# KrishTanna28/Real-Time-Video-Deepfake-Detection

Hardware: AMD Instinct MI355X
Metric: face-crops/sec (224x224 crops through EfficientNet-B0 classify) (higher is better)
Workload: dtype f32; 1 GPU; configs[1]: batch=256 random 224x224 crops, EfficientNet-B0 fp32 inference; batch_per_gpu=256, parallelism=frame-shard x1, no data-path collective, forwards_in_flight=2

## Files before the change

### real-time-video-deepfake-detection_amd/csrc/b0_kernels.h

```cpp
#pragma once
#include <hip/hip_runtime.h>

#include <string>

namespace dfd {

typedef __bf16 bf16_t;

enum Act { ACT_NONE = 0, ACT_SWISH = 1, ACT_RELU = 2, ACT_PRELU = 3 };

template <typename XT>
void launch_stem(const float* x_nchw, const float* w , const float* b,
                 XT* y, int n, hipStream_t s);

template <typename XT>
void launch_stem_dw(const float* x_nchw, const unsigned short* ws3, int plane, int Kp, const float* bs, const float* Wd,
                    const float* bd, XT* Y, float* P, XT* stem_out, int n, int* tiles, hipStream_t s);

void launch_pointwise(const float* X, const float* W, const float* bias, const float* gate,
                      const float* R, float* Y, int M, int K, int N, int HW, int act,
                      hipStream_t s);

struct ConvGeom {
    int H = 0, W = 0, Ho = 0, Wo = 0, Cin = 0, ksize = 1, stride = 1, pad = 0, dil = 1;
// ... 2 lines not shown
bool launch_conv_gemm(const float* X, const float* W, const float* bias, const float* R, float* Y,
                      int n_img, const ConvGeom& g, int Cout, int act, bool res_first, hipStream_t s);

size_t split_weights_count(int N, int K);
void launch_split_weights(const float* W, unsigned short* out, int N, int K, hipStream_t s, bool transposed = false);
bool split_gemm_supports(int K, int N);
bool split_gemm_thin_supports(int K, int N, int HW);
struct S6Table;
S6Table* s6_table_create();
void s6_table_destroy(S6Table* t);
void s6_table_set_force(S6Table* t, int idx);
void s6_table_set_tuning(S6Table* t, bool on);
int s6_table_measured(const S6Table* t);
int s6_max_candidates();
long long s6_chunk_rows(long long M, long long row_bytes, long long HW);
std::string s6_table_export(const S6Table* t);
int s6_table_import(S6Table* t, const char* text, size_t len);
template <typename XT>
bool launch_pointwise_split(S6Table* tab, const XT* X, const unsigned short* W3, const float* bias, const float* gate,
                            const XT* R, XT* Y, int M, int K, int N, int HW, int act, int planes, hipStream_t s);
template <typename XT>
bool launch_conv_gemm_split(S6Table* tab, const XT* X, const unsigned short* W3, const float* bias, const XT* R,
                            XT* Y, int n_img, const ConvGeom& g, int Cout, int act, bool res_first, int planes, hipStream_t s);

template <typename XT>
bool launch_depthwise(const XT* X, const float* W , const float* bias, XT* Y,
                      float* P, int n, int H, int C, int k, int stride, int pad_lo,
                      int* tiles, hipStream_t s);
int depthwise_tiles(int H, int C, int k, int stride);
template <typename XT>
bool launch_mbconv_front(const XT* Xin, int Cin, const unsigned short* We3, int plane, int Kp, const float* Wef, const float* be,
                         const float* Wd, const float* bd, XT* Y, float* P, int n, int H, int C, int k, int stride,
                         int pad_lo, int* tiles, hipStream_t s, bool late = false);
int mbconv_tiles(int H, int C, int k, int stride, int Cin, bool late = false);

void launch_se(const float* P, int tiles, float inv_hw, const float* w1, const float* b1,
               const float* w2t, const float* b2, float* gate, int n, int C, int c_se,
               hipStream_t s);

template <typename XT>
void launch_avgpool(const XT* X, float* Y, int n, int hw, int C, hipStream_t s);
void launch_bf16_to_f32(const bf16_t* x, float* y, size_t n, hipStream_t s);

}
```

### real-time-video-deepfake-detection_amd/csrc/b0_kernels.hip

```cpp
#include "b0_kernels.h"
#include "kernel_util.h"

#include <cstdlib>

namespace dfd {

#ifdef MB_TRACE
__device__ long long g_mb_trace[256];
#define MB_TP(id)                                                                                             \
    do {                                                                                                      \
        if (H == MB_TRACE_H && S == MB_TRACE_S && bid.x == 5 && bid.n == 3 && threadIdx.x == 0 && mtp < 250) { \
            g_mb_trace[mtp++] = (long long)(id);                                                              \
            g_mb_trace[mtp++] = (long long)__builtin_amdgcn_s_memtime();                                      \
        }                                                                                                     \
    } while (0)
#ifndef MB_TRACE_H
#define MB_TRACE_H 56
#endif
#ifndef MB_TRACE_S
#define MB_TRACE_S 1
#endif
extern "C" int dfd_debug_mb_trace(long long* out, int n) {
    return (int)hipMemcpyFromSymbol(out, HIP_SYMBOL(g_mb_trace), (size_t)n * sizeof(long long), 0, hipMemcpyDeviceToHost);
}
// ... 399 lines not shown
    __shared__ v4f wl[K * K * CG];
    __shared__ v4f red[4 * CG];
    const int tid = threadIdx.x;
    const BlkId bid = blk_image_major(tiles_sp * (C / CB));
    const int n = bid.n;
    const int t = bid.x % tiles_sp, chunk = bid.x / tiles_sp;
    const int ty0 = (t / tiles_x) * TH, tx0 = (t % tiles_x) * TW, c0 = chunk * CB;
    const v4f bv = ldg4(bias + c0 + 4 * (tid % CG));
    for (int i = tid; i < K * K * CG; i += 256)
        wl[i] = ldg4(Wt + (size_t)(i / CG) * C + c0 + 4 * (i % CG));
    const int iy0 = ty0 * S - pad_lo, ix0 = tx0 * S - pad_lo;
    const XT* xb = X + (size_t)n * H * H * C + c0;
    constexpr int NEL = IH * IW * CG, NLD = (NEL + 255) / 256;
    v4f stg[NLD];
    bool stg_ok[NLD];
#pragma unroll
    for (int k = 0; k < NLD; ++k) {
        const int i = tid + k * 256 < NEL ? tid + k * 256 : NEL - 1;
        const int cg = i % CG, pix = i / CG;
        const int iy = iy0 + pix / IW, ix = ix0 + pix % IW;
        const bool inside = (unsigned)iy < (unsigned)H && (unsigned)ix < (unsigned)H;
        stg[k] = ld4(xb + ((size_t)(inside ? iy : 0) * H + (inside ? ix : 0)) * C + 4 * cg);
        stg_ok[k] = inside;
    }
#pragma unroll
    for (int k = 0; k < NLD; ++k) {
        const int i = tid + k * 256 < NEL ? tid + k * 256 : NEL - 1;
        tile[i] = stg_ok[k] ? stg[k] : (v4f){0.f, 0.f, 0.f, 0.f};
    }
    __syncthreads();
    dw_compute<K, S, CB, TH, TW, RP, false, XT>(tile, wl, red, bv, Y, P, n, Ho, C, c0, ty0, tx0, t, tiles_sp);
}

template <int K, int S, int CB, int TH, int TW, int RP, int KC, int NSUB, typename XT, int CI>
__global__ __launch_bounds__(256, ((S == 1 && (((TH - 1) * S + K) * ((TW - 1) * S + K) + 63) / 64 * KC > 12) ? 2 : 3)) void mbconv_kernel(const XT* __restrict__ X,
                                                     const float* __restrict__ We,
                                                     const float* __restrict__ be,
                                                     const float* __restrict__ Wt,
                                                     const float* __restrict__ bias,
                                                     XT* __restrict__ Y, float* __restrict__ P,
                                                     int H, int Ho, int C, int Cin, int pad_lo,
                                                     int tiles_x, int tiles_sp) {
    using Sh = DwShape<K, S, CB, TH, TW>;
    constexpr int CG = Sh::CG, IH = Sh::IH, IW = Sh::IW;
    constexpr int NTB = CB / 16;
    constexpr int NP = IH * IW, NMT = (NP + 15) / 16, NIT = (NMT + 3) / 4;
    constexpr int NM = CI / 4;
    static_assert(sizeof(XT) == 4 && CI % 8 == 0 && KC == (NM + 3) / 4, "fp32 activations, compile-time Cin");
    __shared__ v4f tile[IH * IW * CG];
    __shared__ v4f wl[K * K * CG];
    __shared__ v4f red[4 * CG];
    const int tid = threadIdx.x, lane = tid & 63, wave = tid >> 6, j = lane & 15, q = lane >> 4;
    const BlkId bid = blk_image_major(tiles_sp * (C / (CB * NSUB)));
    const int n = bid.n;
    const int t = bid.x % tiles_sp, group = bid.x / tiles_sp;
    const int ty0 = (t / tiles_x) * TH, tx0 = (t % tiles_x) * TW;
    const int iy0 = ty0 * S - pad_lo, ix0 = tx0 * S - pad_lo;
#ifdef MB_TRACE
    int mtp = 0;
#endif
    MB_TP(0);

    const XT* xb = X + (size_t)n * H * H * Cin;
    v4f xf[NIT][KC];
#pragma unroll
    for (int it = 0; it < NIT; ++it) {
        const int p = (wave + 4 * it) * 16 + j;
        const int iy = iy0 + p / IW, ix = ix0 + p % IW;
        const bool inside = p < NP && (unsigned)iy < (unsigned)H && (unsigned)ix < (unsigned)H;
        const float* px = reinterpret_cast<const float*>(xb) + ((size_t)(inside ? iy : 0) * H + (inside ? ix : 0)) * CI + q * NM;
#pragma unroll
        for (int kk = 0; kk < KC; ++kk) {
            v4f v;
            if (NM % 4 == 0 || kk < KC - 1) v = ldg4u(px + 4 * kk);
            else { const v2f t2 = ldg2(px + 4 * kk); v = (v4f){t2.x, t2.y, 0.f, 0.f}; }
            xf[it][kk] = inside ? v : (v4f){0.f, 0.f, 0.f, 0.f};
        }
    }

    static_assert(K * K * CG <= 256, "one depthwise weight vector per thread");
    struct ChunkW { v4f wl, bv, wf[NTB][KC], bex[NTB]; };
    auto load_chunk = [&](int sub, ChunkW& w) {
        const int c0 = (group * NSUB + sub) * CB;
        const int i = tid < K * K * CG ? tid : 0;
        w.wl = ldg4(Wt + (size_t)(i / CG) * C + c0 + 4 * (i % CG));
        w.bv = ldg4(bias + c0 + 4 * (tid % CG));
#pragma unroll
        for (int nt = 0; nt < NTB; ++nt) {
            w.bex[nt] = ldg4(be + c0 + nt * 16 + 4 * q);
#pragma unroll
            for (int kk = 0; kk < KC; ++kk) {
                const float* pw = We + (size_t)(c0 + nt * 16 + j) * CI + q * NM + 4 * kk;
                if (NM % 4 == 0 || kk < KC - 1) w.wf[nt][kk] = ldg4u(pw);
                else { const v2f t2 = ldg2(pw); w.wf[nt][kk] = (v4f){t2.x, t2.y, 0.f, 0.f}; }
            }
        }
    };
    ChunkW cw[2];
    load_chunk(0, cw[0]);
#pragma unroll
    for (int sub = 0; sub < NSUB; ++sub) {
        const int c0 = (group * NSUB + sub) * CB;
        ChunkW& cur = cw[sub & 1];
        MB_TP(1);
        if (sub > 0) __syncthreads();
        MB_TP(2);
        if (tid < K * K * CG) wl[tid] = cur.wl;
        load_chunk(sub + 1 < NSUB ? sub + 1 : NSUB - 1, cw[(sub + 1) & 1]);
        const v4f bv = cur.bv;
        v4f (&wf)[NTB][KC] = cur.wf;
        v4f (&bex)[NTB] = cur.bex;
        MB_TP(3);
#pragma unroll
        for (int it = 0; it < NIT; ++it) {
            const int mt = wave + 4 * it;
            if (mt < NMT) {
                v4f acc[NTB];
#pragma unroll
                for (int nt = 0; nt < NTB; ++nt) acc[nt] = bex[nt];
                if constexpr (NTB == 1) {
                    v4f acc1 = (v4f){0.f, 0.f, 0.f, 0.f};
#pragma unroll
                    for (int i = 0; i < NM; ++i) {
                        if (i & 1) acc1 = __builtin_amdgcn_mfma_f32_16x16x4f32(wf[0][i / 4][i % 4], xf[it][i / 4][i % 4], acc1, 0, 0, 0);
                        else acc[0] = __builtin_amdgcn_mfma_f32_16x16x4f32(wf[0][i / 4][i % 4], xf[it][i / 4][i % 4], acc[0], 0, 0, 0);
                    }
                    acc[0] += acc1;
                } else {
#pragma unroll
                    for (int i = 0; i < NM; ++i)
#pragma unroll
                        for (int nt = 0; nt < NTB; ++nt)
// ... 326 lines not shown
    }
    MB_TP(4);
    __syncthreads();
    MB_TP(5);
    dw_compute<K, S, CB, TH, TW, RP, false, XT>(tile, wl, red, bv, Y, P, n, 112, 32, 0, ty0, tx0, t, tiles_sp);
    MB_TP(6);
#ifdef MB_TRACE
    if (bid.x == 5 && bid.n == 3 && threadIdx.x == 0) g_mb_trace[255] = mtp;
#endif
}

template <typename XT>
void launch_stem_dw(const float* x, const unsigned short* ws3, int plane, int Kp, const float* bs, const float* Wd,
                    const float* bd, XT* Y, float* P, XT* stem_out, int n, int* tiles, hipStream_t s) {
    const int tx = 112 / 16, ty = 112 / 8;
    *tiles = tx * ty;
    hipLaunchKernelGGL(stem_dw_kernel<XT>, dim3(tx * ty * n), dim3(256), 0, s, x, ws3, plane, Kp, bs, Wd, bd, Y, P, stem_out, tx,
                       tx * ty);
}
template void launch_stem_dw<float>(const float*, const unsigned short*, int, int, const float*, const float*, const float*, float*, float*, float*, int, int*, hipStream_t);
template void launch_stem_dw<bf16_t>(const float*, const unsigned short*, int, int, const float*, const float*, const float*, bf16_t*, float*, bf16_t*, int, int*, hipStream_t);

template <int K, int S, int CB, int TH, int TW, int RP, typename XT>
static void dw_launch(const XT* X, const float* W, const float* b, XT* Y, float* P, int n,
                      int H, int C, int pad_lo, int* tiles, hipStream_t s) {
    const int Ho = (H + S - 1) / S;
    const int tx = (Ho + TW - 1) / TW, ty = (Ho + TH - 1) / TH;
    const int tiles_sp = tx * ty;
    *tiles = tiles_sp;
    hipLaunchKernelGGL((dw_kernel<K, S, CB, TH, TW, RP, XT>), dim3(tiles_sp * (C / CB) * n), dim3(256), 0,
                       s, X, W, b, Y, P, H, Ho, C, pad_lo, tx, tiles_sp);
}

template <int K, int S, int CB, int TH, int TW, int RP, int KC, int NSUB, typename XT, int CI>
static void mb_launch(const XT* X, int Cin, const float* We, const float* be, const float* W, const float* b,
                      XT* Y, float* P, int n, int H, int C, int pad_lo, int* tiles, hipStream_t s) {
    const int Ho = (H + S - 1) / S;
    const int tx = (Ho + TW - 1) / TW, ty = (Ho + TH - 1) / TH;
    const int tiles_sp = tx * ty;
    *tiles = tiles_sp;
    hipLaunchKernelGGL((mbconv_kernel<K, S, CB, TH, TW, RP, KC, NSUB, XT, CI>), dim3(tiles_sp * (C / (CB * NSUB)) * n),
                       dim3(256), 0, s, X, We, be, W, b, Y, P, H, Ho, C, Cin, pad_lo, tx, tiles_sp);
}


template <int K, int CPT, typename XT>
__global__ __launch_bounds__(256) void dw_rows7_kernel(const XT* __restrict__ X, const float* __restrict__ Wt,
                                                       const float* __restrict__ bias, XT* __restrict__ Y,
                                                       float* __restrict__ P, int C, int groups) {
    constexpr int H = 7, PAD = (K - 1) / 2, NV = CPT / 4;
    __shared__ v4f red[8 * 32 * NV];
    const BlkId bid = blk_image_major(groups);
    const int tid = threadIdx.x, row = tid >> 5, cl = tid & 31;
    const int c = (bid.x * 32 + cl) * CPT;
    const bool live = row < H && c < C;
    const int cc = c < C ? c : 0, r = row < H ? row : 0;
    const XT* xb = X + (size_t)bid.n * H * H * C + cc;
    v4f acc[H][NV];
#pragma unroll
    for (int v = 0; v < NV; ++v) {
        const v4f bv = ldg4(bias + cc + 4 * v);
#pragma unroll
        for (int ox = 0; ox < H; ++ox) acc[ox][v] = bv;
    }
    constexpr int KY_UNROLL = K == 3 && CPT == 4 ? 3 : (CPT == 4 ? 2 : 1);
#pragma unroll KY_UNROLL
    for (int ky = 0; ky < K; ++ky) {
        const int iy = r + ky - PAD;
        const bool ok = (unsigned)iy < (unsigned)H;
        const XT* xr = xb + (size_t)(ok ? iy : 0) * H * C;
        v4f in[H][NV], w[K][NV];
#pragma unroll
        for (int ix = 0; ix < H; ++ix)
#pragma unroll
            for (int v = 0; v < NV; ++v) in[ix][v] = ld4(xr + (size_t)ix * C + 4 * v);
// ... 447 lines not shown
    }
    if (var == 17 && k == 5 && stride == 1 && H == 28 && C == 240 && Cin == 40) {
        mb2_launch<5, 1, 16, 14, 28, 4, 2, XT, 256, false, 40, 4>(Xin, Cin, We3, plane, Kp, Wef, be, Wd, bd, Y, P, n, H, C, pad_lo, tiles, s);
        return true;
    }
    if (var == 14 && k == 5 && stride == 1 && H == 28 && C == 240 && Cin == 40) {
        mb2_launch<5, 1, 16, 7, 28, 7, 2, XT, 256, false, 40, 4>(Xin, Cin, We3, plane, Kp, Wef, be, Wd, bd, Y, P, n, H, C, pad_lo, tiles, s);
        return true;
    }
    if (var == 13 && k == 3 && stride == 1 && H == 56 && C == 144 && Cin == 24) {
        mb2_launch<3, 1, 16, 14, 28, 7, 1, XT, 256, true, 24, 4>(Xin, Cin, We3, plane, Kp, Wef, be, Wd, bd, Y, P, n, H, C, pad_lo, tiles, s);
        return true;
    }
#ifdef DFD_MB_ABLATION
#define DFD_ABL_CASE(A)                                                                                              \
    if (var == 20 + A && H == 56 && stride == 1) {                                                                  \
        const int tx = 2, ty = 4;                                                                                   \
        *tiles = tx * ty;                                                                                           \
        hipLaunchKernelGGL((mbconv2_kernel<3, 1, 16, 14, 28, 7, 1, XT, A, 256, false, 24>), dim3(tx * ty * (C / 16) * n), dim3(256), 0, s, Xin, \
                           We3, plane, Kp, Wef, be, Wd, bd, Y, P, H, 56, C, Cin, pad_lo, tx, tx * ty);              \
        return true;                                                                                                \
    }                                                                                                               \
    if (var == 20 + A && H == 28 && stride == 1) {                                                                  \
        *tiles = 1;                                                                                                 \
        hipLaunchKernelGGL((mbconv2_kernel<5, 1, 16, 28, 28, 7, 2, XT, A, 256, false, 40>), dim3((C / 16) * n), dim3(256), 0, s, Xin,   \
                           We3, plane, Kp, Wef, be, Wd, bd, Y, P, H, 28, C, Cin, pad_lo, 1, 1);                     \
        return true;                                                                                                \
    }
    DFD_MB2_ABL(DFD_ABL_CASE)
#undef DFD_ABL_CASE
#endif
    return false;
}
template bool launch_mbconv_front<float>(const float*, int, const unsigned short*, int, int, const float*, const float*, const float*, const float*, float*, float*, int, int, int, int, int, int, int*, hipStream_t, bool);
template bool launch_mbconv_front<bf16_t>(const bf16_t*, int, const unsigned short*, int, int, const float*, const float*, const float*, const float*, bf16_t*, float*, int, int, int, int, int, int, int*, hipStream_t, bool);

int mbconv_tiles(int H, int C, int k, int stride, int Cin, bool late) {
    const int Ho = (H + stride - 1) / stride;
    int best = -1;
#define DFD_MB2_TILES(VV, KK, SS, HH, CC, CI, CB, TH, TW, RP, NK)                    \
    if (k == KK && stride == SS && H == HH && C == CC && Cin == CI) {                \
        const int tl = ((Ho + TW - 1) / TW) * ((Ho + TH - 1) / TH);                  \
        if (tl > best) best = tl;                                                    \
    }
    DFD_MB2_TABLE(DFD_MB2_TILES)
#define DFD_MB3_TILES(VV, KK, SS, HH, CC, CI, CB, TH, TW, RP, NK, NT, INS) DFD_MB2_TILES(VV, KK, SS, HH, CC, CI, CB, TH, TW, RP, NK)
    DFD_MB3_TABLE(DFD_MB3_TILES)
#undef DFD_MB3_TILES
#undef DFD_MB2_TILES
#define DFD_MB1_TILES(VV, KK, SS, HH, CC, CI, CB, TH, TW, RP, KC, NSUB)              \
    if (k == KK && stride == SS && H == HH && C == CC && Cin == CI) {                \
        const int tl = ((Ho + TW - 1) / TW) * ((Ho + TH - 1) / TH);                  \
        if (tl > best) best = tl;                                                    \
    }
    DFD_MB1_TABLE(DFD_MB1_TILES)
#undef DFD_MB1_TILES
    if (k == 5 && stride == 1 && H == 28 && C == 240 && Cin == 40 && best < 4) best = 4;
#define DFD_MB_LATE_TILES(KK, SS, HH, CC, CI) \
    if (late && k == KK && stride == SS && H == HH && C == CC && Cin == CI && best < 1) best = 1;
    DFD_MB_LATE_TABLE(DFD_MB_LATE_TILES)
#undef DFD_MB_LATE_TILES
    return best;
}

int depthwise_tiles(int H, int C, int k, int stride) {
    const int Ho = (H + stride - 1) / stride;
// ... 129 lines not shown
```

### real-time-video-deepfake-detection_amd/csrc/b0_plan.hip

```cpp
#include <algorithm>

#include "b0_kernels.h"
#include "dfd_common.h"

namespace dfd {

thread_local std::string g_create_error;

int fail(dfd_handle* h, int code, const char* fmt, ...) {
    char buf[512];
    va_list ap;
    va_start(ap, fmt);
    vsnprintf(buf, sizeof buf, fmt, ap);
    va_end(ap);
    if (h) h->err = buf;
    else g_create_error = buf;
    return code;
}

namespace {

struct Stage { int rep, k, s, e, ci, co; };
const Stage kStages[] = {{1, 3, 1, 1, 32, 16}, {2, 3, 2, 6, 16, 24}, {2, 5, 2, 6, 24, 40},
                         {3, 3, 2, 6, 40, 80}, {3, 5, 1, 6, 80, 112}, {4, 5, 2, 6, 112, 192},
// ... 156 lines not shown
    return pool.emplace(key, key).first->second.c_str();
}

}

template <typename XT>
static int b0_forward_t(dfd_handle* h, const float* x, int n, float* logits_dev, B0Tap* tap, B0Prof* prof) {
    if (n <= 0) return fail(h, DFD_ERR_ARG, "batch must be positive");
    if (n > h->max_batch) return fail(h, DFD_ERR_CAPACITY, "batch %d exceeds handle capacity %d", n, h->max_batch);
    const B0Plan& P = h->b0;
    hipStream_t s = h->stream;
    Marks mk{prof, s};
    int rc;
    XT* const io0 = reinterpret_cast<XT*>(h->io0);
    XT* const io1 = reinterpret_cast<XT*>(h->io1);
    XT* const expbuf = reinterpret_cast<XT*>(h->expbuf);
    XT* const dwbuf = reinterpret_cast<XT*>(h->dwbuf);
    XT* const headbuf = reinterpret_cast<XT*>(h->headbuf);
    mk.mark("start");
    const bool stem_fused = h->fuse_stem && P.blocks[0].expand == 1;
    int stem_tiles = 0;
    if (stem_fused) {
        const bool want_stem = tap && tap->name && std::string(tap->name) == "stem";
        const unsigned short* ws3 = split_weights(h, P.stem_w, 32, 27, true);
        if (!ws3) return DFD_ERR_HIP;
        launch_stem_dw<XT>(x, ws3, (int)split_weights_count(32, 27), 64, P.stem_b, P.blocks[0].dw_w, P.blocks[0].dw_b, dwbuf,
                           h->pool, want_stem ? io0 : (XT*)nullptr, n, &stem_tiles, s);
        mk.mark("b0.dw");
    } else {
        launch_stem<XT>(x, P.stem_w, P.stem_b, io0, n, s);
        mk.mark("stem");
    }
    if ((rc = tap_out(h, tap, "stem", io0, (size_t)n * 112 * 112 * 32))) return rc;
    XT* cur = io0;
    XT* nxt = io1;
    int bi = 0;
    for (const B0Block& b : P.blocks) {
        const int m_in = n * b.h_in * b.h_in, m_out = n * b.h_out * b.h_out;
        const std::string q = "b" + std::to_string(bi);
        const XT* dw_in = cur;
        int tiles = 0;
        bool fused = false;
        const unsigned short* we3 = nullptr;
        const bool late_here = h->fuse_late && !((h->fuse_late_skip >> bi) & 1u);
        if (b.expand != 1 && h->fuse_expand && mbconv_tiles(b.h_in, b.c_exp, b.kernel, b.stride, b.c_in, late_here) > 0 &&
            !(we3 = split_weights(h, b.exp_w, b.c_exp, b.c_in))) return DFD_ERR_HIP;
        if (we3 && launch_mbconv_front<XT>(cur, b.c_in, we3, (int)split_weights_count(b.c_exp, b.c_in), (b.c_in + 63) / 64 * 64,
                                           b.exp_w, b.exp_b, b.dw_w, b.dw_b, dwbuf, h->pool, n, b.h_in, b.c_exp,
                                           b.kernel, b.stride, b.pad_lo, &tiles, s, late_here)) {
            fused = true;
            mk.mark(layer_name(bi, "dw"));
            if (tap && tap->name && q + ".exp" == tap->name)
                return fail(h, DFD_ERR_STATE, "tap '%s': the expanded tensor is not materialised when expand is fused "
                                              "(dfd_set_option(h, \"fuse_expand\", 0))", tap->name);
        }
        if (!fused && b.expand != 1) {
            if ((rc = pointwise_t<XT>(h, cur, b.exp_w, b.exp_b, nullptr, nullptr, expbuf, m_in, b.c_in, b.c_exp,
                                      b.h_in * b.h_in, ACT_SWISH))) return rc;
            mk.mark(layer_name(bi, "exp"));
            if ((rc = tap_out(h, tap, q + ".exp", expbuf, (size_t)m_in * b.c_exp))) return rc;
            dw_in = expbuf;
        }
        if (bi == 0 && stem_fused) {
            tiles = stem_tiles;
        } else if (!fused) {
            if (!launch_depthwise<XT>(dw_in, b.dw_w, b.dw_b, dwbuf, h->pool, n, b.h_in, b.c_exp, b.kernel,
                                      b.stride, b.pad_lo, &tiles, s))
                return fail(h, DFD_ERR_STATE, "no depthwise kernel for block %d", bi);
            mk.mark(layer_name(bi, "dw"));
        }
        if ((rc = tap_out(h, tap, q + ".dw", dwbuf, (size_t)m_out * b.c_exp))) return rc;
        launch_se(h->pool, tiles, 1.0f / (float)(b.h_out * b.h_out), b.se_w1, b.se_b1, b.se_w2, b.se_b2,
                  h->gate, n, b.c_exp, b.c_se, s);
        mk.mark(layer_name(bi, "se"));
        if ((rc = tap_out(h, tap, q + ".gate", h->gate, (size_t)n * b.c_exp))) return rc;
        if ((rc = pointwise_t<XT>(h, dwbuf, b.proj_w, b.proj_b, h->gate, b.skip ? cur : (const XT*)nullptr, nxt, m_out,
                                  b.c_exp, b.c_out, b.h_out * b.h_out, ACT_NONE))) return rc;
        mk.mark(layer_name(bi, "proj"));
        if ((rc = tap_out(h, tap, q + ".out", nxt, (size_t)m_out * b.c_out))) return rc;
        XT* t = cur; cur = nxt; nxt = t;
        ++bi;
    }
    const B0Block& last = P.blocks.back();
    const int hw = last.h_out * last.h_out;
    if ((rc = pointwise_t<XT>(h, cur, P.head_w, P.head_b, nullptr, nullptr, headbuf, n * hw, last.c_out, 1280, hw,
                              ACT_SWISH))) return rc;
    mk.mark("head");
    if ((rc = tap_out(h, tap, "head", headbuf, (size_t)n * hw * 1280))) return rc;
    launch_avgpool<XT>(headbuf, h->feat, n, hw, 1280, s);
    mk.mark("avgpool");
    if ((rc = tap_out(h, tap, "feat", h->feat, (size_t)n * 1280))) return rc;
    if (!logits_dev) return DFD_OK;
    if ((rc = pointwise(h, h->feat, P.fc1_w, P.fc1_b, nullptr, nullptr, h->fc1, n, 1280, 512, 1, ACT_RELU))) return rc;
    if ((rc = pointwise(h, h->fc1, P.fc2_w, P.fc2_b, nullptr, nullptr, h->fc2, n, 512, 256, 1, ACT_RELU))) return rc;
    launch_pointwise(h->fc2, P.fc3_w, P.fc3_b, nullptr, nullptr, logits_dev, n, 256, 1, 1, ACT_NONE, s);
    mk.mark("mlp");
    if ((rc = tap_out(h, tap, "logit", logits_dev, (size_t)n))) return rc;
    DFD_HIP_TRY(h, hipGetLastError());
    return DFD_OK;
}

float* b0_last_block_out(const dfd_handle* h) { return h->b0.blocks.size() % 2 == 0 ? h->io0 : h->io1; }

int b0_head_preact(dfd_handle* h, int n, void* z_out) {
    const B0Plan& P = h->b0;
    const B0Block& last = P.blocks.back();
    const int hw = last.h_out * last.h_out;
    if (h->act_bf16)
        return pointwise_t<bf16_t>(h, reinterpret_cast<const bf16_t*>(b0_last_block_out(h)), P.head_w, P.head_b, nullptr, nullptr,
                                   static_cast<bf16_t*>(z_out), n * hw, last.c_out, 1280, hw, ACT_NONE);
    return pointwise_t<float>(h, b0_last_block_out(h), P.head_w, P.head_b, nullptr, nullptr, static_cast<float*>(z_out),
                              n * hw, last.c_out, 1280, hw, ACT_NONE);
// ... 10 lines not shown
```

### real-time-video-deepfake-detection_amd/csrc/dfd_api.hip

```cpp
#include "b0_kernels.h"
#include "dfd_common.h"

using namespace dfd;

namespace {

int dev_alloc(dfd_handle* h, size_t bytes, float** out) {
    void* p = nullptr;
    DFD_HIP_TRY(h, hipMalloc(&p, bytes ? bytes : 4));
    h->owned.push_back(p);
    *out = static_cast<float*>(p);
    return DFD_OK;
}

__global__ __launch_bounds__(256) void fill_pattern_kernel(float* __restrict__ x, size_t n) {
    const size_t i = (size_t)blockIdx.x * 256 + threadIdx.x;
    if (i >= n) return;
    uint32_t v = (uint32_t)i * 2654435761u;
    v ^= v >> 15; v *= 2246822519u; v ^= v >> 13;
    x[i] = ((float)(v >> 8) * (1.0f / 16777216.0f) - 0.5f) * 4.0f;
}

int create_impl(dfd_handle* h, int device, const void* blob, size_t blob_len, int max_batch) {
    int ndev = 0;
    if (hipGetDeviceCount(&ndev) != hipSuccess || ndev <= 0)
        return fail(h, DFD_ERR_NO_DEVICE, "no HIP device visible (this library has no CPU path)");
    if (device < 0 || device >= ndev) return fail(h, DFD_ERR_ARG, "device %d out of range (0..%d)", device, ndev - 1);
    DFD_HIP_TRY(h, hipSetDevice(device));
    hipDeviceProp_t prop;
    DFD_HIP_TRY(h, hipGetDeviceProperties(&prop, device));
    if (strncmp(prop.gcnArchName, "gfx950", 6) != 0)
        return fail(h, DFD_ERR_NO_DEVICE, "device %d is %s; this library is built for gfx950 only", device, prop.gcnArchName);
    h->device = device;
    h->max_batch = max_batch;
    if (const char* e = getenv("DFD_FUSE_EXPAND")) h->fuse_expand = atoi(e) != 0;
    if (const char* e = getenv("DFD_FUSE_STEM")) h->fuse_stem = atoi(e) != 0;
    if (const char* e = getenv("DFD_FUSE_LATE")) h->fuse_late = atoi(e) != 0;
    if (const char* e = getenv("DFD_FUSE_LATE_SKIP")) h->fuse_late_skip = (unsigned)atoi(e);
    if (const char* e = getenv("DFD_SPLIT_GEMM")) h->split_gemm = atoi(e) != 0;
    if (const char* e = getenv("DFD_BF16_ACTIVATIONS")) h->act_bf16 = atoi(e) != 0;
    if (const char* e = getenv("DFD_JPEG_DEVICE_RESTART")) h->jpeg_device_restart = atoi(e) != 0;
    h->gemm = s6_table_create();
    if (!h->gemm) return fail(h, DFD_ERR_ARG, "out of host memory");
    DFD_HIP_TRY(h, hipStreamCreateWithFlags(&h->stream, hipStreamNonBlocking));
    DFD_HIP_TRY(h, hipEventCreate(&h->ev0));
    DFD_HIP_TRY(h, hipEventCreate(&h->ev1));

    std::string perr;
    if (!parse_blob(blob, blob_len, &h->tensors, &perr)) return fail(h, DFD_ERR_BLOB, "%s", perr.c_str());
    size_t total = 0;
    for (auto& kv : h->tensors) total += (kv.second.count * 4 + 255) / 256 * 256;
    float* wbase = nullptr;
    int rc = dev_alloc(h, total, &wbase);
    if (rc) return rc;
    size_t off = 0;
    for (auto& kv : h->tensors) {
        Tensor& t = kv.second;
        t.dev = reinterpret_cast<float*>(reinterpret_cast<char*>(wbase) + off);
        DFD_HIP_TRY(h, hipMemcpy(t.dev, t.host, t.count * 4, hipMemcpyHostToDevice));
        t.host = nullptr;
        off += (t.count * 4 + 255) / 256 * 256;
    }
    if ((rc = b0_build_plan(h))) return rc;
    if ((rc = color_tables_init(h))) return rc;
    if ((rc = ssd_init(h))) return rc;
    if ((rc = mtcnn_init(h))) return rc;
    if ((rc = haar_init(h))) return rc;

    const B0Plan& P = h->b0;
// ... 60 lines not shown
extern "C" {

int dfd_abi_version(void) { return DFD_ABI_VERSION; }

int dfd_create(int device, const void* blob, size_t blob_len, int max_batch, dfd_handle** out) {
    if (!out) return fail(nullptr, DFD_ERR_ARG, "dfd_create: out is null");
    *out = nullptr;
    if (!blob || max_batch <= 0 || max_batch > 4096)
        return fail(nullptr, DFD_ERR_ARG, "dfd_create: blob is null or max_batch outside 1..4096");
    dfd_handle* h = new (std::nothrow) dfd_handle();
    if (!h) return fail(nullptr, DFD_ERR_ARG, "dfd_create: out of host memory");
    const int rc = create_impl(h, device, blob, blob_len, max_batch);
    if (rc != DFD_OK) {
        g_create_error = h->err;
        destroy_impl(h);
        return rc;
    }
    *out = h;
    return DFD_OK;
}

void dfd_destroy(dfd_handle* h) { destroy_impl(h); }

const char* dfd_last_error(const dfd_handle* h) { return h ? h->err.c_str() : g_create_error.c_str(); }

int dfd_max_batch(const dfd_handle* h) { return h ? h->max_batch : DFD_ERR_ARG; }

int dfd_set_option(dfd_handle* h, const char* name, int value) {
    if (!h || !name) return DFD_ERR_ARG;
    if (strcmp(name, "fuse_expand") == 0) { h->fuse_expand = value != 0; return DFD_OK; }
    if (strcmp(name, "fuse_late") == 0) { h->fuse_late = value != 0; return DFD_OK; }
    if (strcmp(name, "fuse_late_skip") == 0) { h->fuse_late_skip = (unsigned)value; return DFD_OK; }
    if (strcmp(name, "fuse_stem") == 0) { h->fuse_stem = value != 0; return DFD_OK; }
    if (strcmp(name, "split_gemm") == 0) { h->split_gemm = value != 0; return DFD_OK; }
    if (strcmp(name, "mtcnn") == 0) { h->use_mtcnn = value != 0; return DFD_OK; }
    if (strcmp(name, "overlap_forensics") == 0) { h->overlap_forensics = value != 0; return DFD_OK; }
    if (strcmp(name, "bf16_activations") == 0) { h->act_bf16 = value != 0; return DFD_OK; }
    if (strcmp(name, "bf16_weight_planes") == 0) {
        if (value != 1 && value != 3) return fail(h, DFD_ERR_ARG, "bf16_weight_planes must be 1 or 3");
        h->bf16_planes = value;
        return DFD_OK;
    }
    if (strcmp(name, "gemm_tile") == 0) { s6_table_set_force(h->gemm, value); return DFD_OK; }
    if (strcmp(name, "jpeg_device_entropy") == 0) { h->jpeg_device_entropy = value < 0 ? 0 : value; return DFD_OK; }
    if (strcmp(name, "jpeg_device_restart") == 0) { h->jpeg_device_restart = value != 0; return DFD_OK; }
    if (strcmp(name, "jpeg_rounds") == 0) { h->jpeg_rounds = value; return DFD_OK; }
    if (strcmp(name, "jpeg_chunk_bytes") == 0) {
        if (value < 256 || value > (1 << 20) || (value & (value - 1))) return fail(h, DFD_ERR_ARG, "jpeg_chunk_bytes: a power of two in 256 .. 2^20");
        h->jpeg_chunk_bytes = value;
        return DFD_OK;
    }
    if (strcmp(name, "stream_priority") == 0) {
        if (value < -1 || value > 1) return fail(h, DFD_ERR_ARG, "stream_priority must be -1, 0 or 1");
        DFD_HIP_TRY(h, hipSetDevice(h->device));
        DFD_HIP_TRY(h, stream_sync(h));
        if (h->aux_stream) DFD_HIP_TRY(h, hipStreamSynchronize(h->aux_stream));
        if (h->copy_stream) DFD_HIP_TRY(h, hipStreamSynchronize(h->copy_stream));
        int least = 0, greatest = 0;
        DFD_HIP_TRY(h, hipDeviceGetStreamPriorityRange(&least, &greatest));
        const int prio = value > 0 ? greatest : (value < 0 ? least : (least + greatest) / 2);
        hipStream_t fresh = nullptr;
        DFD_HIP_TRY(h, hipStreamCreateWithPriority(&fresh, hipStreamNonBlocking, prio));
        hipStreamDestroy(h->stream);
        h->stream = fresh;
        return DFD_OK;
    }
    if (strcmp(name, "profile_stride") == 0) { h->prof_stride = value > 0 ? value : 1; return DFD_OK; }
    return fail(h, DFD_ERR_ARG, "unknown option '%s'", name);
}

int dfd_warmup(dfd_handle* h, int n_crops, int n_frames) {
    if (!h) return DFD_ERR_ARG;
    if (n_crops < 0 || n_crops > h->max_batch || n_frames < 0)
        return fail(h, DFD_ERR_ARG, "warmup: n_crops outside 0..%d or n_frames negative", h->max_batch);
    DFD_HIP_TRY(h, hipSetDevice(h->device));
    s6_table_set_tuning(h->gemm, true);
    int rc = DFD_OK;
    if (n_crops > 0) {
        const size_t cnt = (size_t)n_crops * 3 * 224 * 224;
        hipLaunchKernelGGL(fill_pattern_kernel, dim3((unsigned)((cnt + 255) / 256)), dim3(256), 0, h->stream, h->in_nchw, cnt);
        rc = b0_forward(h, h->in_nchw, n_crops, h->logits, nullptr, nullptr);
    }
    if (rc == DFD_OK && n_frames > 0) rc = ssd_warmup(h, n_frames);
    s6_table_set_tuning(h->gemm, false);
    if (rc) return rc;
    DFD_HIP_TRY(h, stream_sync(h));
    return DFD_OK;
}

int dfd_classifier_crop_count(const dfd_handle* h, unsigned long long* total) {
    if (!h || !total) return DFD_ERR_ARG;
    *total = h->classifier_crops;
    return DFD_OK;
}

int dfd_jpeg_decode_counts(const dfd_handle* h, unsigned long long* on_device, unsigned long long* on_host) {
    if (!h || !on_device || !on_host) return DFD_ERR_ARG;
    *on_device = h->jpeg_frames_device;
    *on_host = h->jpeg_frames_host;
    return DFD_OK;
}

int dfd_gemm_tile_count(void) { return s6_max_candidates(); }

int dfd_tiles_export(dfd_handle* h, char* text_out, size_t capacity, size_t* length) {
    if (!h || !length) return DFD_ERR_ARG;
    const std::string t = s6_table_export(h->gemm);
    *length = t.size();
    if (!text_out) return DFD_OK;
    if (t.size() > capacity) return fail(h, DFD_ERR_ARG, "tiles_export: %zu bytes needed, capacity %zu", t.size(), capacity);
    memcpy(text_out, t.data(), t.size());
    return DFD_OK;
}

int dfd_tiles_import(dfd_handle* h, const char* text, size_t length, int* accepted) {
    if (!h || (!text && length)) return DFD_ERR_ARG;
    const int n = s6_table_import(h->gemm, text, length);
// ... 161 lines not shown
```

### real-time-video-deepfake-detection_amd/csrc/dfd_common.h

```cpp
#pragma once
#include <hip/hip_runtime.h>

#include <cstdarg>
#include <cstdint>
#include <cstdio>
#include <cstring>
#include <map>
#include <string>
#include <vector>

#include "../../include/dfd_hip.h"
#include "blob_reader.h"
#include "imgproc_kernels.h"

namespace dfd {

struct ForensicState;
void forensic_destroy(dfd_handle* h);
struct FreqState;
void freq_destroy(dfd_handle* h);
struct SsdState;
int ssd_init(dfd_handle* h);
void ssd_destroy(dfd_handle* h);
int ssd_warmup(dfd_handle* h, int n_frames);
// ... 57 lines not shown
    bool overlap_forensics = true;
    hipStream_t copy_stream = nullptr;
    hipEvent_t copy_done[2] = {nullptr, nullptr}, slot_free[2] = {nullptr, nullptr};
    dfd::DevBuf stage[2];
    std::map<std::string, dfd::Tensor> tensors;
    std::vector<void*> owned;
    dfd::B0Plan b0;
    float *in_nchw = nullptr, *io0 = nullptr, *io1 = nullptr, *expbuf = nullptr, *dwbuf = nullptr;
    float *pool = nullptr, *gate = nullptr, *headbuf = nullptr, *feat = nullptr, *fc1 = nullptr,
          *fc2 = nullptr, *logits = nullptr;
    dfd::ColorTables color{};
    bool has_color = false;
    dfd::DevBuf frame_buf, lab_buf, crop_buf, lut_buf, desc_buf, u8_out, face_batch;
    dfd::DevBuf det_desc;
    int last_detections = 0;
    std::vector<char> crop_valid;
    int n_compact = 0;
    bool tta_armed = false;
    int tta_copies = 0, tta_capacity = 0;
    std::vector<dfd_tta_draw> tta_draws;
    std::vector<float> tta_logits;
    int tta_out_faces = 0, tta_out_copies = 0;
    dfd::DevBuf tta_desc, tta_logit_buf;
    unsigned long long classifier_crops = 0;
    dfd::ForensicState* forensic = nullptr;
    dfd::FreqState* freq = nullptr;
    dfd::SsdState* ssd = nullptr;
    dfd::MtcnnState* mtcnn = nullptr;
    dfd::HaarState* haar = nullptr;
    dfd::CommState* comm = nullptr;
    bool use_mtcnn = true;
    bool fuse_stem = true;
    bool fuse_expand = true;
    bool fuse_late = true;
    unsigned fuse_late_skip = (1u << 8) | (1u << 9);
    bool split_gemm = true;
    bool act_bf16 = false;
    int bf16_planes = 3;
    dfd::DevBuf jpeg_work;
    dfd::DevBuf jpeg_raw[2];
    dfd::DevBuf jpeg_work2[2];
    hipStream_t jpeg_stream = nullptr;
    hipEvent_t jpeg_done[2] = {nullptr, nullptr}, frames_free[2] = {nullptr, nullptr};
    void* jpeg_host = nullptr;
    size_t jpeg_host_cap = 0;
    int jpeg_device_entropy = 2;
    int jpeg_device_restart = 0;
    int jpeg_rounds = 16;
    int jpeg_chunk_bytes = 512;
    unsigned long long jpeg_frames_device = 0, jpeg_frames_host = 0;
    dfd::DevBuf tap_buf;
    std::map<const float*, unsigned short*> wsplit;
    dfd::S6Table* gemm = nullptr;
    dfd::B0Prof prof;
    int prof_steps = 0;
    int prof_seen = 0, prof_stride = 1;
    std::string err;
};

namespace dfd {

extern thread_local std::string g_create_error;

int fail(dfd_handle* h, int code, const char* fmt, ...);

#define DFD_HIP_TRY(h, expr)                                                                    \
// ... 69 lines not shown
```

Before: 94380 crops/s.

## Fuse block 0 projection into block 1 expand+depthwise kernel

Adds a PROJ0 variant of the mbconv front kernel that reads block 0's depthwise output, applies the SE gate and the 32->16 projection with bf16 split MFMAs in registers, then runs block 1's expand and depthwise directly. This removes the separate block 0 projection launch and the write and re-read of its 112x112x16 output. In exchange, the 32-channel input is reloaded for every halo tile and the projection is recomputed on overlapping pixels. The path is skipped during warmup so GEMM tuning still sees the unfused projection.

Measured after the change: 97290 crops/s (median of 6 runs). 3.1% higher.

```diff
diff --git a/real-time-video-deepfake-detection_amd/csrc/b0_kernels.h b/real-time-video-deepfake-detection_amd/csrc/b0_kernels.h
--- a/real-time-video-deepfake-detection_amd/csrc/b0_kernels.h
+++ b/real-time-video-deepfake-detection_amd/csrc/b0_kernels.h
@@ -58,6 +58,10 @@
 bool launch_mbconv_front(const XT* Xin, int Cin, const unsigned short* We3, int plane, int Kp, const float* Wef, const float* be,
                          const float* Wd, const float* bd, XT* Y, float* P, int n, int H, int C, int k, int stride,
                          int pad_lo, int* tiles, hipStream_t s, bool late = false);
+bool mbconv_proj0_supported(int H, int C, int k, int stride, int Cin, int C0);
+bool launch_mbconv_front_proj0(const float* Xdw0, const float* gate0, const unsigned short* Wp3, int plane, int Kp, const float* bp,
+                               const float* Wef, const float* be, const float* Wd, const float* bd, float* Y, float* P, int n,
+                               int H, int C, int k, int stride, int Cin, int pad_lo, int* tiles, hipStream_t s);
 int mbconv_tiles(int H, int C, int k, int stride, int Cin, bool late = false);
 
 void launch_se(const float* P, int tiles, float inv_hw, const float* w1, const float* b1,
diff --git a/real-time-video-deepfake-detection_amd/csrc/b0_kernels.hip b/real-time-video-deepfake-detection_amd/csrc/b0_kernels.hip
--- a/real-time-video-deepfake-detection_amd/csrc/b0_kernels.hip
+++ b/real-time-video-deepfake-detection_amd/csrc/b0_kernels.hip
@@ -455,7 +455,17 @@
     dw_compute<K, S, CB, TH, TW, RP, false, XT>(tile, wl, red, bv, Y, P, n, Ho, C, c0, ty0, tx0, t, tiles_sp);
 }
 
-template <int K, int S, int CB, int TH, int TW, int RP, int KC, int NSUB, typename XT, int CI>
+template <bool PROJ0>
+struct Proj0Args {};
+template <>
+struct Proj0Args<true> {
+    const float* gate;
+    const unsigned short* W3;
+    const float* bias;
+    int plane, Kp;
+};
+
+template <int K, int S, int CB, int TH, int TW, int RP, int KC, int NSUB, typename XT, int CI, bool PROJ0 = false>
 __global__ __launch_bounds__(256, ((S == 1 && (((TH - 1) * S + K) * ((TW - 1) * S + K) + 63) / 64 * KC > 12) ? 2 : 3)) void mbconv_kernel(const XT* __restrict__ X,
                                                      const float* __restrict__ We,
                                                      const float* __restrict__ be,
@@ -463,7 +473,7 @@
                                                      const float* __restrict__ bias,
                                                      XT* __restrict__ Y, float* __restrict__ P,
                                                      int H, int Ho, int C, int Cin, int pad_lo,
-                                                     int tiles_x, int tiles_sp) {
+                                                     int tiles_x, int tiles_sp, const Proj0Args<PROJ0> pj) {
     using Sh = DwShape<K, S, CB, TH, TW>;
     constexpr int CG = Sh::CG, IH = Sh::IH, IW = Sh::IW;
     constexpr int NTB = CB / 16;
@@ -484,23 +494,6 @@
 #endif
     MB_TP(0);
 
-    const XT* xb = X + (size_t)n * H * H * Cin;
-    v4f xf[NIT][KC];
-#pragma unroll
-    for (int it = 0; it < NIT; ++it) {
-        const int p = (wave + 4 * it) * 16 + j;
-        const int iy = iy0 + p / IW, ix = ix0 + p % IW;
-        const bool inside = p < NP && (unsigned)iy < (unsigned)H && (unsigned)ix < (unsigned)H;
-        const float* px = reinterpret_cast<const float*>(xb) + ((size_t)(inside ? iy : 0) * H + (inside ? ix : 0)) * CI + q * NM;
-#pragma unroll
-        for (int kk = 0; kk < KC; ++kk) {
-            v4f v;
-            if (NM % 4 == 0 || kk < KC - 1) v = ldg4u(px + 4 * kk);
-            else { const v2f t2 = ldg2(px + 4 * kk); v = (v4f){t2.x, t2.y, 0.f, 0.f}; }
-            xf[it][kk] = inside ? v : (v4f){0.f, 0.f, 0.f, 0.f};
-        }
-    }
-
     static_assert(K * K * CG <= 256, "one depthwise weight vector per thread");
     struct ChunkW { v4f wl, bv, wf[NTB][KC], bex[NTB]; };
     auto load_chunk = [&](int sub, ChunkW& w) {
@@ -520,7 +513,66 @@
         }
     };
     ChunkW cw[2];
-    load_chunk(0, cw[0]);
+
+    v4f xf[NIT][KC];
+    if constexpr (PROJ0) {
+        static_assert(CI == 16 && KC == 1, "block 0's projection: 32 -> 16 channels, one 16-channel row tile");
+        constexpr int C0 = 32;
+        const float* xb = reinterpret_cast<const float*>(X) + (size_t)n * H * H * C0 + 8 * q;
+        v4f raw[NIT][2];
+#pragma unroll
+        for (int it = 0; it < NIT; ++it) {
+            const int p = (wave + 4 * it) * 16 + j;
+            const int iy = iy0 + p / IW, ix = ix0 + p % IW;
+            const bool inside = p < NP && (unsigned)iy < (unsigned)H && (unsigned)ix < (unsigned)H;
+            const float* px = xb + ((size_t)(inside ? iy : 0) * H + (inside ? ix : 0)) * C0;
+            raw[it][0] = ldg4(px);
+            raw[it][1] = ldg4(px + 4);
+        }
+        const v4f g0 = ldg4(pj.gate + (size_t)n * C0 + 8 * q), g1 = ldg4(pj.gate + (size_t)n * C0 + 8 * q + 4);
+        const unsigned short* wrow = pj.W3 + (size_t)j * pj.Kp + 8 * q;
+        const bf8 w0 = *reinterpret_cast<const bf8*>(wrow), w1 = *reinterpret_cast<const bf8*>(wrow + (size_t)pj.plane),
+                  w2 = *reinterpret_cast<const bf8*>(wrow + 2 * (size_t)pj.plane);
+        const v4f pb = ldg4(pj.bias + 4 * q);
+        load_chunk(0, cw[0]);
+        bf8 xs[NIT][3];
+#pragma unroll
+        for (int it = 0; it < NIT; ++it) {
+            v4f lo = raw[it][0] * g0, hi = raw[it][1] * g1;
+            asm("" : "+v"(lo), "+v"(hi));
+            split8(lo, hi, xs[it][0], xs[it][1], xs[it][2]);
+        }
+        v4f pacc[NIT];
+#pragma unroll
+        for (int it = 0; it < NIT; ++it) pacc[it] = (v4f){0.f, 0.f, 0.f, 0.f};
+        const bf8* wsel[6] = {&w2, &w1, &w0, &w1, &w0, &w0};
+        const int xsel[6] = {0, 1, 2, 0, 1, 0};
+#pragma unroll
+        for (int p6 = 0; p6 < 6; ++p6)
+#pragma unroll
+            for (int it = 0; it < NIT; ++it)
+                pacc[it] = __builtin_amdgcn_mfma_f32_16x16x32_bf16(*wsel[p6], xs[it][xsel[p6]], pacc[it], 0, 0, 0);
+#pragma unroll
+        for (int it = 0; it < NIT; ++it) xf[it][0] = (pacc[it] + pb) + (v4f){0.f, 0.f, 0.f, 0.f};
+    } else {
+    const XT* xb = X + (size_t)n * H * H * Cin;
+#pragma unroll
+    for (int it = 0; it < NIT; ++it) {
+        const int p = (wave + 4 * it) * 16 + j;
+        const int iy = iy0 + p / IW, ix = ix0 + p % IW;
+        const bool inside = p < NP && (unsigned)iy < (unsigned)H && (unsigned)ix < (unsigned)H;
+        const float* px = reinterpret_cast<const float*>(xb) + ((size_t)(inside ? iy : 0) * H + (inside ? ix : 0)) * CI + q * NM;
+#pragma unroll
+        for (int kk = 0; kk < KC; ++kk) {
+            v4f v;
+            if (NM % 4 == 0 || kk < KC - 1) v = ldg4u(px + 4 * kk);
+            else { const v2f t2 = ldg2(px + 4 * kk); v = (v4f){t2.x, t2.y, 0.f, 0.f}; }
+            xf[it][kk] = inside ? v : (v4f){0.f, 0.f, 0.f, 0.f};
+        }
+    }
+    }
+
+    if constexpr (!PROJ0) load_chunk(0, cw[0]);
 #pragma unroll
     for (int sub = 0; sub < NSUB; ++sub) {
         const int c0 = (group * NSUB + sub) * CB;
@@ -913,15 +965,16 @@
                        s, X, W, b, Y, P, H, Ho, C, pad_lo, tx, tiles_sp);
 }
 
-template <int K, int S, int CB, int TH, int TW, int RP, int KC, int NSUB, typename XT, int CI>
+template <int K, int S, int CB, int TH, int TW, int RP, int KC, int NSUB, typename XT, int CI, bool PROJ0 = false>
 static void mb_launch(const XT* X, int Cin, const float* We, const float* be, const float* W, const float* b,
-                      XT* Y, float* P, int n, int H, int C, int pad_lo, int* tiles, hipStream_t s) {
+                      XT* Y, float* P, int n, int H, int C, int pad_lo, int* tiles, hipStream_t s,
+                      const Proj0Args<PROJ0> pj = Proj0Args<PROJ0>{}) {
     const int Ho = (H + S - 1) / S;
     const int tx = (Ho + TW - 1) / TW, ty = (Ho + TH - 1) / TH;
     const int tiles_sp = tx * ty;
     *tiles = tiles_sp;
-    hipLaunchKernelGGL((mbconv_kernel<K, S, CB, TH, TW, RP, KC, NSUB, XT, CI>), dim3(tiles_sp * (C / (CB * NSUB)) * n),
-                       dim3(256), 0, s, X, We, be, W, b, Y, P, H, Ho, C, Cin, pad_lo, tx, tiles_sp);
+    hipLaunchKernelGGL((mbconv_kernel<K, S, CB, TH, TW, RP, KC, NSUB, XT, CI, PROJ0>), dim3(tiles_sp * (C / (CB * NSUB)) * n),
+                       dim3(256), 0, s, X, We, be, W, b, Y, P, H, Ho, C, Cin, pad_lo, tx, tiles_sp, pj);
 }
 
 
@@ -1435,6 +1488,18 @@
 #endif
     return false;
 }
+bool mbconv_proj0_supported(int H, int C, int k, int stride, int Cin, int C0) {
+    return k == 3 && stride == 2 && H == 112 && C == 96 && Cin == 16 && C0 == 32 && mb_variant(H, stride) == -2;
+}
+bool launch_mbconv_front_proj0(const float* Xdw0, const float* gate0, const unsigned short* Wp3, int plane, int Kp, const float* bp,
+                               const float* Wef, const float* be, const float* Wd, const float* bd, float* Y, float* P, int n,
+                               int H, int C, int k, int stride, int Cin, int pad_lo, int* tiles, hipStream_t s) {
+    if (!mbconv_proj0_supported(H, C, k, stride, Cin, 32)) return false;
+    const Proj0Args<true> pj{gate0, Wp3, bp, plane, Kp};
+    mb_launch<3, 2, 32, 8, 8, 2, 1, 3, float, 16, true>(Xdw0, Cin, Wef, be, Wd, bd, Y, P, n, H, C, pad_lo, tiles, s, pj);
+    return true;
+}
+
 template bool launch_mbconv_front<float>(const float*, int, const unsigned short*, int, int, const float*, const float*, const float*, const float*, float*, float*, int, int, int, int, int, int, int*, hipStream_t, bool);
 template bool launch_mbconv_front<bf16_t>(const bf16_t*, int, const unsigned short*, int, int, const float*, const float*, const float*, const float*, bf16_t*, float*, int, int, int, int, int, int, int*, hipStream_t, bool);
 
diff --git a/real-time-video-deepfake-detection_amd/csrc/b0_plan.hip b/real-time-video-deepfake-detection_amd/csrc/b0_plan.hip
--- a/real-time-video-deepfake-detection_amd/csrc/b0_plan.hip
+++ b/real-time-video-deepfake-detection_amd/csrc/b0_plan.hip
@@ -212,6 +212,14 @@
         mk.mark("stem");
     }
     if ((rc = tap_out(h, tap, "stem", io0, (size_t)n * 112 * 112 * 32))) return rc;
+    bool proj0 = false;
+    if constexpr (sizeof(XT) == 4) {
+        const B0Block &p0 = P.blocks[0], &p1 = P.blocks[1];
+        proj0 = h->fuse_proj0 && h->fuse_expand && h->split_gemm && !h->warming && p0.expand == 1 && !p0.skip &&
+                p0.c_out >= 16 && split_gemm_supports(p0.c_exp, p0.c_out) &&
+                mbconv_proj0_supported(p1.h_in, p1.c_exp, p1.kernel, p1.stride, p1.c_in, p0.c_exp) &&
+                !(tap && tap->name && std::string(tap->name) == "b0.out");
+    }
     XT* cur = io0;
     XT* nxt = io1;
     int bi = 0;
@@ -219,11 +227,29 @@
         const int m_in = n * b.h_in * b.h_in, m_out = n * b.h_out * b.h_out;
         const std::string q = "b" + std::to_string(bi);
         const XT* dw_in = cur;
+        XT* dw_out = dwbuf;
         int tiles = 0;
         bool fused = false;
         const unsigned short* we3 = nullptr;
+        if constexpr (sizeof(XT) == 4) {
+            if (proj0 && bi == 1) {
+                const B0Block& p0 = P.blocks[0];
+                const unsigned short* wp3 = split_weights(h, p0.proj_w, p0.c_out, p0.c_exp);
+                if (!wp3) return DFD_ERR_HIP;
+                dw_out = expbuf;
+                if (!launch_mbconv_front_proj0(dwbuf, h->gate, wp3, (int)split_weights_count(p0.c_out, p0.c_exp),
+                                               (p0.c_exp + 63) / 64 * 64, p0.proj_b, b.exp_w, b.exp_b, b.dw_w, b.dw_b, dw_out,
+                                               h->pool, n, b.h_in, b.c_exp, b.kernel, b.stride, b.c_in, b.pad_lo, &tiles, s))
+                    return fail(h, DFD_ERR_STATE, "no fused projection kernel for block 1");
+                fused = true;
+                mk.mark(layer_name(bi, "dw"));
+                if (tap && tap->name && q + ".exp" == tap->name)
+                    return fail(h, DFD_ERR_STATE, "tap '%s': the expanded tensor is not materialised when expand is fused "
+                                                  "(dfd_set_option(h, \"fuse_expand\", 0))", tap->name);
+            }
+        }
         const bool late_here = h->fuse_late && !((h->fuse_late_skip >> bi) & 1u);
-        if (b.expand != 1 && h->fuse_expand && mbconv_tiles(b.h_in, b.c_exp, b.kernel, b.stride, b.c_in, late_here) > 0 &&
+        if (!fused && b.expand != 1 && h->fuse_expand && mbconv_tiles(b.h_in, b.c_exp, b.kernel, b.stride, b.c_in, late_here) > 0 &&
             !(we3 = split_weights(h, b.exp_w, b.c_exp, b.c_in))) return DFD_ERR_HIP;
         if (we3 && launch_mbconv_front<XT>(cur, b.c_in, we3, (int)split_weights_count(b.c_exp, b.c_in), (b.c_in + 63) / 64 * 64,
                                            b.exp_w, b.exp_b, b.dw_w, b.dw_b, dwbuf, h->pool, n, b.h_in, b.c_exp,
@@ -249,15 +275,17 @@
                 return fail(h, DFD_ERR_STATE, "no depthwise kernel for block %d", bi);
             mk.mark(layer_name(bi, "dw"));
         }
-        if ((rc = tap_out(h, tap, q + ".dw", dwbuf, (size_t)m_out * b.c_exp))) return rc;
+        if ((rc = tap_out(h, tap, q + ".dw", dw_out, (size_t)m_out * b.c_exp))) return rc;
         launch_se(h->pool, tiles, 1.0f / (float)(b.h_out * b.h_out), b.se_w1, b.se_b1, b.se_w2, b.se_b2,
                   h->gate, n, b.c_exp, b.c_se, s);
         mk.mark(layer_name(bi, "se"));
         if ((rc = tap_out(h, tap, q + ".gate", h->gate, (size_t)n * b.c_exp))) return rc;
-        if ((rc = pointwise_t<XT>(h, dwbuf, b.proj_w, b.proj_b, h->gate, b.skip ? cur : (const XT*)nullptr, nxt, m_out,
-                                  b.c_exp, b.c_out, b.h_out * b.h_out, ACT_NONE))) return rc;
-        mk.mark(layer_name(bi, "proj"));
-        if ((rc = tap_out(h, tap, q + ".out", nxt, (size_t)m_out * b.c_out))) return rc;
+        if (!(proj0 && bi == 0)) {
+            if ((rc = pointwise_t<XT>(h, dw_out, b.proj_w, b.proj_b, h->gate, b.skip ? cur : (const XT*)nullptr, nxt, m_out,
+                                      b.c_exp, b.c_out, b.h_out * b.h_out, ACT_NONE))) return rc;
+            mk.mark(layer_name(bi, "proj"));
+            if ((rc = tap_out(h, tap, q + ".out", nxt, (size_t)m_out * b.c_out))) return rc;
+        }
         XT* t = cur; cur = nxt; nxt = t;
         ++bi;
     }
diff --git a/real-time-video-deepfake-detection_amd/csrc/dfd_api.hip b/real-time-video-deepfake-detection_amd/csrc/dfd_api.hip
--- a/real-time-video-deepfake-detection_amd/csrc/dfd_api.hip
+++ b/real-time-video-deepfake-detection_amd/csrc/dfd_api.hip
@@ -35,6 +35,7 @@
     h->max_batch = max_batch;
     if (const char* e = getenv("DFD_FUSE_EXPAND")) h->fuse_expand = atoi(e) != 0;
     if (const char* e = getenv("DFD_FUSE_STEM")) h->fuse_stem = atoi(e) != 0;
+    if (const char* e = getenv("DFD_FUSE_PROJ0")) h->fuse_proj0 = atoi(e) != 0;
     if (const char* e = getenv("DFD_FUSE_LATE")) h->fuse_late = atoi(e) != 0;
     if (const char* e = getenv("DFD_FUSE_LATE_SKIP")) h->fuse_late_skip = (unsigned)atoi(e);
     if (const char* e = getenv("DFD_SPLIT_GEMM")) h->split_gemm = atoi(e) != 0;
@@ -161,6 +162,7 @@
     if (strcmp(name, "fuse_late") == 0) { h->fuse_late = value != 0; return DFD_OK; }
     if (strcmp(name, "fuse_late_skip") == 0) { h->fuse_late_skip = (unsigned)value; return DFD_OK; }
     if (strcmp(name, "fuse_stem") == 0) { h->fuse_stem = value != 0; return DFD_OK; }
+    if (strcmp(name, "fuse_proj0") == 0) { h->fuse_proj0 = value != 0; return DFD_OK; }
     if (strcmp(name, "split_gemm") == 0) { h->split_gemm = value != 0; return DFD_OK; }
     if (strcmp(name, "mtcnn") == 0) { h->use_mtcnn = value != 0; return DFD_OK; }
     if (strcmp(name, "overlap_forensics") == 0) { h->overlap_forensics = value != 0; return DFD_OK; }
@@ -204,6 +206,7 @@
         return fail(h, DFD_ERR_ARG, "warmup: n_crops outside 0..%d or n_frames negative", h->max_batch);
     DFD_HIP_TRY(h, hipSetDevice(h->device));
     s6_table_set_tuning(h->gemm, true);
+    h->warming = true;
     int rc = DFD_OK;
     if (n_crops > 0) {
         const size_t cnt = (size_t)n_crops * 3 * 224 * 224;
@@ -212,6 +215,7 @@
     }
     if (rc == DFD_OK && n_frames > 0) rc = ssd_warmup(h, n_frames);
     s6_table_set_tuning(h->gemm, false);
+    h->warming = false;
     if (rc) return rc;
     DFD_HIP_TRY(h, stream_sync(h));
     return DFD_OK;
diff --git a/real-time-video-deepfake-detection_amd/csrc/dfd_common.h b/real-time-video-deepfake-detection_amd/csrc/dfd_common.h
--- a/real-time-video-deepfake-detection_amd/csrc/dfd_common.h
+++ b/real-time-video-deepfake-detection_amd/csrc/dfd_common.h
@@ -113,6 +113,8 @@
     bool use_mtcnn = true;
     bool fuse_stem = true;
     bool fuse_expand = true;
+    bool fuse_proj0 = true;
+    bool warming = false;
     bool fuse_late = true;
     unsigned fuse_late_skip = (1u << 8) | (1u << 9);
     bool split_gemm = true;
```
